# HAHHHD/mllp

Hardware: AMD Instinct MI355X
Metric: LP instances/sec (fwd+bwd) on Netlib batch; achieved HBM GB/s on CSR SpMM (higher is better)
Workload: dtype f32; 1 GPU; netlib_full: BASELINE.json configs[2], 97 instances / 1,074,147 nnz per global batch, one block-diagonal batch per GPU, one Adam step per global batch: fwd + BCE + bwd + gradient all-reduce + Adam, fp32; global_batch=97, instances_rank0=97, nnz_rank0=1074147, hip_graph=False, parallelism=dp1

## Files before the change

### mllp_amd/csrc/fused_kernels.hip

```cpp
#include <algorithm>
#include <vector>

#include "device_utils.h"
#include "host_graph.h"
#include "internal.h"
#include "node_bodies.h"

namespace mllp {

typedef float f32x4m __attribute__((ext_vector_type(4)));

#ifdef MLLP_TIMING_BUILD
static int g_fused_abl = [] {
    const char* e = getenv("MLLP_FUSED_ABL");
    return e ? atoi(e) : 0;
}();
#define FUSED_ABL(bit) ((J.abl & (bit)) != 0)
__device__ unsigned long long g_fused_stamps[8192 * 8];
__device__ unsigned long long g_fused_stamps1[8192 * 8];
#define FUSED_STAMP(k)                                                                      \
    {                                                                                       \
        __builtin_amdgcn_sched_barrier(0);                                                  \
        const unsigned long long now_ = __builtin_amdgcn_s_memtime();                       \
        __builtin_amdgcn_sched_barrier(0);                                                  \
// ... 1399 lines not shown
        }
    }
    const float x = J.x_dst[rowc];
    const float Zn = J.Z[rowc];
    const float4 ax = reinterpret_cast<const float4*>(J.aux)[rowc];
    {
        float* rt = tiles + 64 * G1S + lane * R1S;
        rt[0] = writer ? x : 0.0f;
        rt[1] = writer ? Zn : 0.0f;
        rt[2] = writer ? 1.0f : 0.0f;
        rt[3] = writer ? ax.w : 0.0f;
        rt[4] = writer ? ax.x : 0.0f;
    }
    const float Dn = gv * Zn + gb * ax.w + ge * ax.x;
    const float cc = gb - Dn;
    const float qp = fmaf(W.pq, x, W.pq0), t = fmaf(W.pt, x, W.pt0);
    float ds = 0.0f, dt = 0.0f, dq = 0.0f;
    const int n_mine = slot_count(r);
    FUSED_STAMP(1)
    for (int k0 = 0; __any(k0 < n_mine); k0 += 8) {
        Ent8 N;
        const bool more = __any(k0 + 8 < n_mine);
        if (more) ent8_load(J.s, r, k0 + 8, N);
#define MLLP_BWD1_SLOT(K, E_)                                                              \
    {                                                                                      \
        const float l_ = fmaf(qp, E_.y, E_.x * t);                                         \
        const float al_ = (K) < n_mine ? exp_acc(l_ - ax.y) * ax.z : 0.0f;                 \
        const float dl_ = al_ * fmaf(gv, E_.y, fmaf(E_.x, ge, cc));                        \
        ds += dl_;                                                                         \
        dt = fmaf(dl_, E_.x, dt);                                                          \
        dq = fmaf(dl_, E_.y, dq);                                                          \
    }
        MLLP_BWD1_SLOT(k0, E.e0)
        MLLP_BWD1_SLOT(k0 + 1, E.e1)
        MLLP_BWD1_SLOT(k0 + 2, E.e2)
        MLLP_BWD1_SLOT(k0 + 3, E.e3)
        if (__any(k0 + 4 < n_mine)) {
            MLLP_BWD1_SLOT(k0 + 4, E.e4)
            MLLP_BWD1_SLOT(k0 + 5, E.e5)
            MLLP_BWD1_SLOT(k0 + 6, E.e6)
            MLLP_BWD1_SLOT(k0 + 7, E.e7)
        }
#undef MLLP_BWD1_SLOT
        if (more) E = N;
    }
    FUSED_STAMP(2)
    if (r.mode >= 1) {
        ds = shared_sum1(ds, r.mode); dt = shared_sum1(dt, r.mode); dq = shared_sum1(dq, r.mode);
    }
    if (r.mode == 3) {
        const int wave = threadIdx.x >> 6;
        if (lane == 0) *reinterpret_cast<float4*>(merge_lds + wave * 4) = make_float4(ds, dt, dq, 0.0f);
        __syncthreads();
        float a = 0.0f, b = 0.0f, c = 0.0f;
        for (int w = 0; w < FW; ++w) {
            const float4 v = lds4(merge_lds + w * 4);
            a += v.x; b += v.y; c += v.z;
        }
        ds = a; dt = b; dq = c;
        __syncthreads();
        if (threadIdx.x >= 64) return;
    }
    if (writer) {
        accS[0] = fmaf(dq, x, accS[0]);
        accS[1] += dq;
        accS[2] = fmaf(ds, x, accS[2]);
        accS[3] = fmaf(dt, x, accS[3]);
        accS[4] += ds;
        accS[5] += dt;
    }
    FUSED_STAMP(3)
    const int kq = lane >> 4, rr = lane & 15;
    const float* gt = tiles + kq * G1S + rr;
    const float* rt = tiles + 64 * G1S + kq * R1S + rr;
#pragma unroll
    for (int s = 0; s < 16; ++s) {
        const float a = gt[4 * s * G1S];
        const float b = rr < 5 ? rt[4 * s * R1S] : 0.0f;
        accT = __builtin_amdgcn_mfma_f32_16x16x4f32(a, b, accT, 0, 0, 0);
    }
    FUSED_STAMP(4)
}

__global__ __launch_bounds__(FT) void fused_bwd1_kernel(BwdLaunch1 A) {
    __shared__ BwdW1 Ws_[MAXJOBS];
    __shared__ float merge_lds[FW * 4];
    __shared__ float tiles_[FW * TILE1];
    const int tid = threadIdx.x, lane = tid & 63, wave = tid >> 6;
    for (int j = 0; j < A.n_jobs; ++j) {
        const BwdJob1& J = A.job[j];
        BwdW1& W = Ws_[j];
        if (tid < 16) { W.wv[tid] = J.p.Wv[tid]; W.bv[tid] = J.p.bv[tid]; W.we[tid] = J.p.we[tid]; }
        if (tid == 0) { W.pq = J.D[OFF_PQ]; W.pq0 = J.D[OFF_PQ0]; W.pt = J.D[OFF_PT]; W.pt0 = J.D[OFF_PT0]; }
    }
    __syncthreads();
    float* tiles = tiles_ + wave * TILE1;
    const BlockPart B = block_part();
#ifdef MLLP_TIMING_BUILD
    unsigned long long stamp_sum[8] = {0, 0, 0, 0, 0, 0, 0, 0};
    unsigned long long stamp_last = __builtin_amdgcn_s_memtime();
    const unsigned long long stamp_begin = stamp_last;
#define STAMP_ARGS1 , stamp_sum, stamp_last
#else
#define STAMP_ARGS1
#endif
    for (int j = 0; j < A.n_jobs; ++j) {
        const BwdJob1& J = A.job[j];
        const PartTiers P = J.s.part[B.px];
        f32x4m accT = splat4(0.0f);
        float accS[6] = {0.0f, 0.0f, 0.0f, 0.0f, 0.0f, 0.0f};
        for (int k = B.bi; k < P.n_block; k += B.gp)
            bwd1_row(J, Ws_[j], block_slot<1>(J.s, P.row0 + k, tid), lane, merge_lds, tiles, accT, accS STAMP_ARGS1);
        WaveList wl = wave_list(J.s, B.px, B.gw);
        for (int c0 = 0; c0 < wl.L; c0 += 64) {
            wave_list_chunk(wl, c0, lane);
            int it = wave_list_get(wl, 0);
            SlotReq q = item_request<1>(J.s, P, max(it, 0), lane);
            for (int k = 0; it >= 0; ++k) {
                const int itn = wave_list_get(wl, k + 1);
                const RowSlot r = slot_make(q);
                q = item_request<1>(J.s, P, max(itn, 0), lane);
                bwd1_row(J, Ws_[j], r, lane, merge_lds, tiles, accT, accS STAMP_ARGS1);
#ifdef MLLP_TIMING_BUILD
                stamp_sum[7] += 1;
#endif
                it = itn;
            }
        }
        __syncthreads();
        float* red = tiles_;
#pragma unroll
        for (int q = 0; q < 4; ++q) red[wave * 262 + ((lane >> 4) * 4 + q) * 16 + (lane & 15)] = accT[q];
#pragma unroll
        for (int i = 0; i < 6; ++i) {
            const float v = wave_sum(accS[i]);
            if (lane == 0) red[wave * 262 + 256 + i] = v;
        }
        __syncthreads();
        float* dst = J.stats + (size_t)blockIdx.x * STAT_FLOATS;
        for (int i = tid; i < STAT_FLOATS; i += FT) dst[i] = 0.0f;
        __syncthreads();
        if (tid < 262) {
            float v = 0.0f;
            for (int w = 0; w < FW; ++w) v += red[w * 262 + tid];
            const int o = tid >> 4, n = tid & 15;
            if (tid >= 256) {
                const int i = tid - 256;
                const int slot = i == 0 ? 768 : i == 1 ? 1024 : i == 2 ? 1280 : i == 3 ? 1280 + 16 : i == 4 ? 1536 : 1536 + 16;
                dst[slot] = v;
            } else if (n == 0) dst[o * 16] = v;
            else if (n == 1) dst[256 + o * 16] = v;
            else if (n < 5) dst[512 + o * 16 + (n - 2)] = v;
        }
        __syncthreads();
#ifdef MLLP_TIMING_BUILD
        stamp_last = __builtin_amdgcn_s_memtime();
#endif
    }
#ifdef MLLP_TIMING_BUILD
    if (lane == 0) {
        stamp_sum[6] = __builtin_amdgcn_s_memtime() - stamp_begin;
        unsigned long long* d = g_fused_stamps1 + (size_t)(blockIdx.x * FW + wave) * 8;
        for (int k = 0; k < 8; ++k) d[k] = stamp_sum[k];
    }
#endif
#undef STAMP_ARGS1
}

__global__ __launch_bounds__(RT) void fused_head_bwd_kernel(int n, const float* __restrict__ h3, const float* __restrict__ fcw,
                                                            const float* __restrict__ dlogits, const int* __restrict__ perm,
                                                            float* __restrict__ dh3, float* __restrict__ head_part) {
    __shared__ float head_lds[(RT / 64) * 18];
    const int tid = threadIdx.x, lane = tid & 63, part = lane & 3;
    HeadAcc ha;
    ha.w = f4zero(); ha.b = 0.0f; ha.l = 0.0f;
    const float4 fw = ld4(fcw + 4 * part);
    for (int row = blockIdx.x * (RT / 4) + (tid >> 2); row < n; row += gridDim.x * (RT / 4)) {
        const float dz = dlogits[perm[row]];
        const float4 hv = ld4(h3 + (size_t)row * 16 + 4 * part);
        *reinterpret_cast<float4*>(dh3 + (size_t)row * 16 + 4 * part) = f4scale(fw, dz);
        fma4(dz, hv, ha.w);
        if (part == 0) ha.b += dz;
    }
    head_partials_store<RT / 64>(ha, head_lds, head_part, tid);
}

struct ReduceArgs {
    const float* stats[MODEL_CONVS];
    float* out[MODEL_CONVS];
    int nblk;
    const float* head_part;
    float* head_out;
    float* loss_out;
};

__device__ __forceinline__ void fused_reduce_body(const ReduceArgs& A, int n_conv) {
    __shared__ float sh[32][32];
    const int tid = threadIdx.x;
    if ((int)blockIdx.x == n_conv * STAT_TILES) {
        if (!A.head_part) return;
        const int col = tid & 31, slice = tid >> 5;
        float v = 0.0f;
        if (col < 18)
            for (int b = slice; b < A.nblk; b += 32) v += A.head_part[(size_t)b * 18 + col];
        sh[slice][col] = v;
        __syncthreads();
        if (tid < 18) {
            float t = 0.0f;
            for (int q = 0; q < 32; ++q) t += sh[q][tid];
            if (tid < 17) A.head_out[tid] = t;
            else if (A.loss_out) A.loss_out[0] = t;
        }
        return;
    }
    float* sh4 = &sh[0][0];
    const int col = tid & 255, slice = tid >> 8;
    const int c = blockIdx.x / STAT_TILES, tile = blockIdx.x % STAT_TILES;
    const float* src = A.stats[c] + tile * 256 + col;
    float v = 0.0f;
    int b = slice;
    for (; b + 124 < A.nblk; b += 128) {
        float t[32];
#pragma unroll
        for (int q = 0; q < 32; ++q) t[q] = src[(size_t)(b + 4 * q) * STAT_FLOATS];
#pragma unroll
        for (int q = 0; q < 32; ++q) v += t[q];
    }
    for (; b + 28 < A.nblk; b += 32) {
        float t[8];
#pragma unroll
        for (int q = 0; q < 8; ++q) t[q] = src[(size_t)(b + 4 * q) * STAT_FLOATS];
#pragma unroll
        for (int q = 0; q < 8; ++q) v += t[q];
    }
    for (; b < A.nblk; b += 4) v += src[(size_t)b * STAT_FLOATS];
    sh4[slice * 256 + col] = v;
    __syncthreads();
    if (tid < 256) A.out[c][tile * 256 + tid] = (sh4[tid] + sh4[256 + tid]) + (sh4[512 + tid] + sh4[768 + tid]);
}
__global__ __launch_bounds__(RT) void fused_reduce_kernel(ReduceArgs A, int n_conv) { fused_reduce_body(A, n_conv); }

struct TailArgs {
    ReduceArgs R;
    ConvParams p[MODEL_CONVS];
    int cin[MODEL_CONVS];
    float* grads[MODEL_CONVS];
    float* zero;
    int n_zero;
    float* params; const float* grads_all; float* m; float* v; float* state;
    float eps;
    int n_params;
    float* D[MODEL_CONVS];
    unsigned long long* sync;
    unsigned* err;
};
__device__ __forceinline__ bool tail_barrier(unsigned long long* cnt, unsigned long long target, unsigned* err_host) {
    __shared__ int ok_s;
    unsigned long long* err_dev = cnt + 2;
    __syncthreads();
    if (threadIdx.x == 0) {
        __threadfence();
        __hip_atomic_fetch_add(cnt, 1ull, __ATOMIC_RELEASE, __HIP_MEMORY_SCOPE_AGENT);
        int spins = 0;
        while (__hip_atomic_load(cnt, __ATOMIC_ACQUIRE, __HIP_MEMORY_SCOPE_AGENT) < target && ++spins < (1 << 22))
            __builtin_amdgcn_s_sleep(8);
        if (spins >= (1 << 22)) {
            __hip_atomic_store(err_dev, 1ull, __ATOMIC_RELAXED, __HIP_MEMORY_SCOPE_AGENT);
            __hip_atomic_store(err_host, 1u, __ATOMIC_RELAXED, __HIP_MEMORY_SCOPE_SYSTEM);
        }
        __threadfence();
        ok_s = __hip_atomic_load(err_dev, __ATOMIC_RELAXED, __HIP_MEMORY_SCOPE_AGENT) == 0ull;
    }
    __syncthreads();
    return ok_s != 0;
}
__global__ __launch_bounds__(RT) void fused_tail_kernel(TailArgs A, int n_conv) {
    const unsigned long long G = gridDim.x, epoch = A.sync[1];
    const int b = blockIdx.x;
    const float step = A.state[0] + 1.0f, lr = A.state[1], b1 = A.state[2], b2 = A.state[3];
    fused_reduce_body(A.R, n_conv);
    if (!tail_barrier(A.sync, (epoch + 1) * G, A.err)) return;
    if (b < n_conv) {
        finalize_conv_body(A.cin[b], A.p[b], A.R.out[b], 1, A.grads[b]);
        __syncthreads();
        const int off = (int)(A.grads[b] - A.grads_all), n = 4 * FEAT * A.cin[b] + 5 * FEAT;
        adam_slice(A.params + off, A.grads_all + off, A.m + off, A.v + off, step, lr, b1, b2, A.eps, 1.0f, n);
        __syncthreads();
        if (threadIdx.x < BLOCK) param_prep_body(A.p[b], A.cin[b], A.D[b]);
    } else if (b == n_conv) {
        for (int k = threadIdx.x; k < A.n_zero; k += RT) A.zero[k] = 0.0f;
        const int off = (int)(A.R.head_out - A.grads_all);
        adam_slice(A.params + off, A.grads_all + off, A.m + off, A.v + off, step, lr, b1, b2, A.eps, 1.0f, A.n_params - off);
        if (threadIdx.x == 0) {
            A.state[0] = step;
            A.sync[1] = epoch + 1;
        }
    }
}

__global__ __launch_bounds__(256) void fused_fill_kernel(int n_dst, const int* __restrict__ perm, const int* __restrict__ ptr,
                                                         const int* __restrict__ idx, const float* __restrict__ val,
                                                         const int* __restrict__ inv_src, const int* __restrict__ sptr,
                                                         int2* __restrict__ sent) {
    const int k = blockIdx.x * 4 + (threadIdx.x >> 6), lane = threadIdx.x & 63;
    if (k >= n_dst) return;
    const int r = perm[k], beg = ptr[r], deg = ptr[r + 1] - beg, o = sptr[k];
    for (int e = lane; e < deg; e += 64) sent[o + e] = make_int2(inv_src[idx[beg + e]], __float_as_int(val[beg + e]));
}
__global__ void fused_permute_kernel(int n, const int* __restrict__ perm, const float* __restrict__ src, float* __restrict__ dst) {
    for (int i = blockIdx.x * blockDim.x + threadIdx.x; i < n; i += gridDim.x * blockDim.x) dst[i] = src[perm[i]];
}
__global__ void fused_pregather_kernel(int64_t nnz, const int2* __restrict__ sent, const float* __restrict__ xs,
                                       float2* __restrict__ sax) {
    for (int64_t e = blockIdx.x * (int64_t)blockDim.x + threadIdx.x; e < nnz; e += (int64_t)gridDim.x * blockDim.x) {
        const int2 v = sent[e];
        sax[e] = make_float2(__int_as_float(v.y), xs[v.x]);
    }
}

#ifdef MLLP_TIMING_BUILD
extern "C" int mllp_timing_read_stamps(unsigned long long* host, int n) {
    return hipMemcpyFromSymbol(host, HIP_SYMBOL(g_fused_stamps), (size_t)n * sizeof(unsigned long long)) == hipSuccess ? 0 : -1;
}
extern "C" int mllp_timing_read_stamps1(unsigned long long* host, int n) {
    return hipMemcpyFromSymbol(host, HIP_SYMBOL(g_fused_stamps1), (size_t)n * sizeof(unsigned long long)) == hipSuccess ? 0 : -1;
}
#endif

template <class T>
static int dev_alloc(mllp_graph* g, size_t count, T** out, const T* host = nullptr, size_t room = 1) {
    void* p = nullptr;
    MLLP_HIP_TRY(hipMalloc(&p, std::max<size_t>(count, room) * sizeof(T)));
    if (count < room) MLLP_HIP_TRY(hipMemset(p, 0, room * sizeof(T)));
    g->allocs.push_back(p);
    if (host && count) MLLP_HIP_TRY(hipMemcpy(p, host, count * sizeof(T), hipMemcpyHostToDevice));
    *out = static_cast<T*>(p);
    return MLLP_OK;
}

static void set_tiers(FusedTiersDev& d, const FusedTiers& t) {
    d.n_block = t.n_block; d.n_wave = t.n_wave; d.n_group = t.n_group; d.n_base = t.n_base;
}

int fused_refill_values(mllp_graph* g, hipStream_t s) {
    int rc;
    if (g->M > 0) {
        hipLaunchKernelGGL(fused_fill_kernel, dim3((unsigned)((g->M + 3) / 4)), dim3(256), 0, s, (int)g->M, g->perm_c, g->A.ptr,
                           g->A.idx, g->A.val, g->inv_v, g->FA.sptr, reinterpret_cast<int2*>(g->FA.sent));
        if ((rc = check_launch("fused_fill A"))) return rc;
    }
    if (g->N > 0) {
        hipLaunchKernelGGL(fused_fill_kernel, dim3((unsigned)((g->N + 3) / 4)), dim3(256), 0, s, (int)g->N, g->perm_v, g->At.ptr,
                           g->At.idx, g->At.val, g->inv_c, g->FAt.sptr, reinterpret_cast<int2*>(g->FAt.sent));
        if ((rc = check_launch("fused_fill At"))) return rc;
    }
    return MLLP_OK;
}

int fused_graph_build(mllp_graph* g, const int* h_csr_ptr, const int* h_csc_ptr) {
    if (g->fused_built) return MLLP_OK;
    if ((int64_t)g->h_csr_ptr.size() != g->M + 1 && !h_csr_ptr) return fail(MLLP_EINVAL, "fused path: no host row pointers");
    HostFusedOrient hc, hv;
    {
#ifdef MLLP_SCALAR_PARTITION
        const std::vector<int> part = host_partition_instances(host_instance_cost(h_csr_ptr, g->h_inst_ptr_m),
                                                               host_instance_cost(h_csc_ptr, g->h_inst_ptr_n), FUSED_PARTS);
#else
        const std::vector<int> part = host_partition_instances_v(host_instance_loads(h_csr_ptr, g->h_inst_ptr_m),
                                                                 host_instance_loads(h_csc_ptr, g->h_inst_ptr_n), FUSED_PARTS);
#endif
        host_build_fused_orient(h_csr_ptr, (int)g->M, g->h_inst_ptr_m, part, &hc);
        host_build_fused_orient(h_csc_ptr, (int)g->N, g->h_inst_ptr_n, part, &hv);
    }
    int rc;
    if ((rc = dev_alloc(g, (size_t)g->M, &g->perm_c, hc.perm.data()))) return rc;
    if ((rc = dev_alloc(g, (size_t)g->N, &g->perm_v, hv.perm.data()))) return rc;
    if ((rc = dev_alloc(g, (size_t)g->M, &g->inv_c, hc.inv.data()))) return rc;
    if ((rc = dev_alloc(g, (size_t)g->N, &g->inv_v, hv.inv.data()))) return rc;
    FusedOrient& A = g->FA;
    FusedOrient& At = g->FAt;
    A.n_dst = (int)g->M; A.n_src = (int)g->N; A.nnz = (int)g->nnz;
    At.n_dst = (int)g->N; At.n_src = (int)g->M; At.nnz = (int)g->nnz;
    for (int q = 0; q < NP; ++q) {
        set_tiers(A.t16[q], hc.t16[q]); set_tiers(A.t1[q], hc.t1[q]);
        set_tiers(At.t16[q], hv.t16[q]); set_tiers(At.t1[q], hv.t1[q]);
    }
    for (int q = 0; q <= NP; ++q) { A.row0[q] = hc.row0[q]; At.row0[q] = hv.row0[q]; }
    {
        const int gp = fused_grid(g) / NP;
        const HostFusedOrient* ho[2] = {&hc, &hv};
        FusedOrient* dv[2] = {&A, &At};
        for (int k = 0; k < 2; ++k) {
            HostWaveLists l16, l16x2, l1;
            host_build_wave_lists(*ho[k], false, gp * FW, FW, 4, &l16);
            host_build_wave_lists(*ho[k], false, 2 * gp * FW, FW, 2, &l16x2);
            host_build_wave_lists(*ho[k], true, gp * FW, FW, 8, &l1);
            FusedOrient& d = *dv[k];
            d.L16 = l16.L; d.nw16 = l16.waves_per_part;
            d.L16x2 = l16x2.L; d.nw16x2 = l16x2.waves_per_part;
            d.L1 = l1.L; d.nw1 = l1.waves_per_part;
            if ((rc = dev_alloc(g, l16.order.size(), &d.lst16, l16.order.data()))) return rc;
            if ((rc = dev_alloc(g, l16x2.order.size(), &d.lst16x2, l16x2.order.data()))) return rc;
            if ((rc = dev_alloc(g, l1.order.size(), &d.lst1, l1.order.data()))) return rc;
        }
    }
    if ((rc = dev_alloc(g, (size_t)g->M + 1, &A.sptr, hc.sptr.data(), 2))) return rc;
    if ((rc = dev_alloc(g, (size_t)g->N + 1, &At.sptr, hv.sptr.data(), 2))) return rc;
    if ((rc = dev_alloc(g, (size_t)g->nnz * 2, &A.sent, (const int*)nullptr, 2))) return rc;
    if ((rc = dev_alloc(g, (size_t)g->nnz * 2, &At.sent, (const int*)nullptr, 2))) return rc;
    if ((rc = dev_alloc(g, (size_t)g->nnz * 2, &A.sax, (const float*)nullptr, 2))) return rc;
    if ((rc = dev_alloc(g, (size_t)g->nnz * 2, &At.sax, (const float*)nullptr, 2))) return rc;
    if ((rc = dev_alloc(g, (size_t)g->N, &g->inv_n_p))) return rc;
    if ((rc = dev_alloc(g, (size_t)g->N, &g->x1_p))) return rc;
    if ((rc = dev_alloc(g, (size_t)g->M, &g->x2_p))) return rc;
    if ((rc = dev_alloc(g, (size_t)g->N, &g->labels_p))) return rc;
    if (!g->tail_sync) {
        if ((rc = dev_alloc(g, (size_t)4, &g->tail_sync))) return rc;
        MLLP_HIP_TRY(hipMemset(g->tail_sync, 0, 32));
        MLLP_HIP_TRY(hipHostMalloc((void**)&g->tail_err_host, 64, hipHostMallocMapped));
        *g->tail_err_host = 0u;
        MLLP_HIP_TRY(hipHostGetDevicePointer((void**)&g->tail_err_dev, g->tail_err_host, 0));
    }
    if ((rc = fused_refill_values(g, 0))) return rc;
    if (g->N > 0) {
        hipLaunchKernelGGL(fused_permute_kernel, dim3(256), dim3(256), 0, 0, (int)g->N, g->perm_v, g->inv_n, g->inv_n_p);
        if ((rc = check_launch("fused_permute inv_n"))) return rc;
    }
    MLLP_HIP_TRY(hipDeviceSynchronize());
    g->fused_built = true;
    return MLLP_OK;
}

int fused_bind(mllp_graph* g, const float* x1, const float* x2, const float* labels, hipStream_t s) {
    int rc;
    hipStreamCaptureStatus cap = hipStreamCaptureStatusNone;
    (void)hipStreamIsCapturing(s, &cap);
    const bool capturing = cap != hipStreamCaptureStatusNone;
    if (capturing) g->bind_captured = true;
    if (g->bind_captured) g->bound_x1 = g->bound_x2 = g->bound_labels = nullptr;
    if (x1 != g->bound_x1 || x2 != g->bound_x2) {
        if (g->N > 0) hipLaunchKernelGGL(fused_permute_kernel, dim3(256), dim3(256), 0, s, (int)g->N, g->perm_v, x1, g->x1_p);
        if (g->M > 0) hipLaunchKernelGGL(fused_permute_kernel, dim3(256), dim3(256), 0, s, (int)g->M, g->perm_c, x2, g->x2_p);
        if (g->nnz > 0) {
            hipLaunchKernelGGL(fused_pregather_kernel, dim3(1024), dim3(256), 0, s, g->nnz,
                               reinterpret_cast<const int2*>(g->FA.sent), g->x1_p, reinterpret_cast<float2*>(g->FA.sax));
            hipLaunchKernelGGL(fused_pregather_kernel, dim3(1024), dim3(256), 0, s, g->nnz,
                               reinterpret_cast<const int2*>(g->FAt.sent), g->x2_p, reinterpret_cast<float2*>(g->FAt.sax));
        }
        if ((rc = check_launch("fused_bind inputs"))) return rc;
        if (!capturing) { g->bound_x1 = x1; g->bound_x2 = x2; }
    }
    if (labels && labels != g->bound_labels) {
        if (g->N > 0) hipLaunchKernelGGL(fused_permute_kernel, dim3(256), dim3(256), 0, s, (int)g->N, g->perm_v, labels, g->labels_p);
        if ((rc = check_launch("fused_bind labels"))) return rc;
        if (!capturing) g->bound_labels = labels;
    }
    return MLLP_OK;
}

int fused_grid(const mllp_graph* g) { return std::max(std::min(g->n_cu, STAT_BLOCKS_MAX) / NP, 1) * NP; }

static FwdJob16 fwd_job16(const FusedOrient& o, const FusedModel& m, int c, const float* x_src, const float* x_dst, float* h) {
    const ConvWs& w = m.w.c[c];
    FwdJob16 J = {};
    J.s = items_dev(o, 0);
    J.x_src = x_src; J.x_dst = x_dst; J.D = w.derived; J.p = conv_params_at(conv_at(m.P, c), MODEL_CONV[c].cin);
    J.h = h; J.Z = w.Z; J.aux = w.aux;
    J.head = 0;
#ifdef MLLP_TIMING_BUILD
    J.abl = g_fused_abl;
#endif
    return J;
}
static FwdJob1 fwd_job1(const FusedOrient& o, const FusedModel& m, int c, const float* x_dst, float* h) {
    const ConvWs& w = m.w.c[c];
    FwdJob1 J = {};
    J.s = items_dev(o, 1);
    J.x_dst = x_dst; J.D = w.derived; J.p = conv_params_at(conv_at(m.P, c), MODEL_CONV[c].cin);
    J.h = h; J.Z = w.Z; J.aux = w.aux;
    return J;
}

static FwdJob16 l3_fwd_job(const mllp_graph* g, const FusedModel& m, int head_mode) {
    const ModelWs& w = m.w;
    FwdJob16 J = fwd_job16(g->FAt, m, CONV_3V, w.h2c, w.h2v, w.h3v);
    J.head = head_mode;
    J.fcw = m.P + OFF_FC; J.fcb = m.P + OFF_FC + FEAT; J.inv_n = g->inv_n_p; J.labels = g->labels_p; J.perm = g->perm_v;
    J.inv_batch = m.inv_batch;
    J.logits = m.logits; J.head_part = w.head_partials;
    return J;
}

int fused_forward(mllp_graph* g, const FusedModel& m, int head_mode, hipStream_t s, bool skip_prep) {
    const int G = fused_grid(g);
    const ModelWs& w = m.w;
    int rc;
    if ((rc = fused_bind(g, m.x1, m.x2, head_mode == 2 ? m.labels : nullptr, s))) return rc;
    if (!skip_prep && (rc = model_param_prep(m.P, w, s))) return rc;
    {
        FwdLaunch1 L = {};
        L.n_jobs = 2;
        L.job[0] = fwd_job1(g->FAt, m, CONV_1V, g->x1_p, w.h1v);
        L.job[1] = fwd_job1(g->FA, m, CONV_1C, g->x2_p, w.h1c);
        hipLaunchKernelGGL(fused_fwd1_kernel, dim3(G), dim3(FT), 0, s, L);
// ... 45 lines not shown
static SrcJob16 src_job16(const FusedOrient& o_src_major, const ConvWs& w, const float* x_rows, float* dx, const float* add) {
    SrcJob16 J = {};
    J.s = items_dev(o_src_major, 2);
    J.x = x_rows; J.rec = w.rec; J.dx = dx;
    J.addp = add ? add : x_rows; J.addw = add ? 1.0f : 0.0f; J.mask = 1;
    return J;
}
static BwdJob1 bwd_job1(const FusedOrient& o, const FusedModel& m, int c, const float* x_dst, const float* g_masked) {
    const ConvWs& w = m.w.c[c];
    BwdJob1 J = {};
    J.s = items_dev(o, 1);
    J.x_dst = x_dst; J.D = w.derived; J.p = conv_params_at(conv_at(m.P, c), MODEL_CONV[c].cin);
    J.g = g_masked; J.Z = w.Z; J.aux = w.aux; J.stats = w.stats;
    return J;
}

int fused_backward(const mllp_graph* g, const FusedModel& m, bool premasked, float* grads, float* loss, hipStream_t s,
                   const FusedAdam* adam) {
    const int G = fused_grid(g);
    const ModelWs& w = m.w;
    int rc;
    const FusedOrient& A = g->FA;
    const FusedOrient& At = g->FAt;
    if (premasked) {
        L3Job L = {};
        L.f = l3_fwd_job(g, m, 2);
        L.rec = w.c[CONV_3V].rec; L.dx_dst = w.d2v; L.stats = w.c[CONV_3V].stats;
        hipLaunchKernelGGL(fused_l3_kernel, dim3(G), dim3(FT), 0, s, L);
        if ((rc = check_launch("fused_l3"))) return rc;
    } else {
        BwdLaunch16 L = {};
        L.n_jobs = 1;
        L.job[0] = bwd_job16(At, m, CONV_3V, w.h2c, w.h2v, w.h3v, w.d3v, nullptr, w.d2v, true, true);
        hipLaunchKernelGGL(fused_bwd16_kernel, dim3(G), dim3(FT), 0, s, L);
        if ((rc = check_launch("fused_bwd16 C3"))) return rc;
    }
    {
        SrcLaunch16 S = {};
        S.n_jobs = 1;
        S.job[0] = src_job16(A, w.c[CONV_3V], w.h2c, w.d2c, nullptr);
        hipLaunchKernelGGL(fused_src16_kernel, dim3(2 * G), dim3(FT), 0, s, S);
        if ((rc = check_launch("fused_src16 C3"))) return rc;
        BwdLaunch16 L = {};
        L.n_jobs = 1;
        L.job[0] = bwd_job16(At, m, CONV_2V, w.h1c, w.h1v, nullptr, w.d2v, nullptr, w.d1v, true, true);
        hipLaunchKernelGGL(fused_bwd16_kernel, dim3(G), dim3(FT), 0, s, L);
        if ((rc = check_launch("fused_bwd16 C2V"))) return rc;
    }
    {
        BwdLaunch16 L = {};
        L.n_jobs = 1;
        L.job[0] = bwd_job16(A, m, CONV_2C, w.h1v, w.h1c, nullptr, w.d2c, nullptr, w.d1c, true, true);
        hipLaunchKernelGGL(fused_bwd16_kernel, dim3(G), dim3(FT), 0, s, L);
        if ((rc = check_launch("fused_bwd16 C2C"))) return rc;
        SrcLaunch16 S = {};
        S.n_jobs = 2;
        S.job[0] = src_job16(A, w.c[CONV_2V], w.h1c, w.d1c_b, w.d1c);
        S.job[1] = src_job16(At, w.c[CONV_2C], w.h1v, w.d1v_b, w.d1v);
        hipLaunchKernelGGL(fused_src16_kernel, dim3(2 * G), dim3(FT), 0, s, S);
        if ((rc = check_launch("fused_src16 C2V + C2C"))) return rc;
    }
    {
        BwdLaunch1 L = {};
        L.n_jobs = 2;
        L.job[0] = bwd_job1(A, m, CONV_1C, g->x2_p, w.d1c_b);
        L.job[1] = bwd_job1(At, m, CONV_1V, g->x1_p, w.d1v_b);
        hipLaunchKernelGGL(fused_bwd1_kernel, dim3(G), dim3(FT), 0, s, L);
        if ((rc = check_launch("fused_bwd1"))) return rc;
    }
    ReduceArgs R = {};
    for (int c = 0; c < MODEL_CONVS; ++c) { R.stats[c] = w.c[c].stats; R.out[c] = w.c[c].red; }
    R.nblk = G;
    R.head_part = w.head_partials;
    R.head_out = grads + OFF_FC;
    R.loss_out = loss;
    if (adam) {
        TailArgs T = {};
        T.R = R;
        for (int c = 0; c < MODEL_CONVS; ++c) {
            T.p[c] = conv_params_at(conv_at(m.P, c), MODEL_CONV[c].cin);
            T.cin[c] = MODEL_CONV[c].cin;
            T.grads[c] = conv_at(grads, c);
            T.D[c] = w.c[c].derived;
        }
        T.zero = grads + OFF_UNUSED;
        T.n_zero = LEN_UNUSED;
        T.params = adam->params; T.grads_all = grads; T.m = adam->m; T.v = adam->v; T.state = adam->state;
        T.eps = adam->eps;
        T.n_params = adam->n;
        T.sync = g->tail_sync;
        T.err = g->tail_err_dev;
        if (g->tail_err_host && *(volatile unsigned*)g->tail_err_host != 0u)
            return fail(MLLP_EHIP, "the grid barrier of fused_tail_kernel timed out in an earlier step (the device was shared with "
                                   "other work): parameters and optimizer state since then are invalid; recreate the graph");
        hipLaunchKernelGGL(fused_tail_kernel, dim3(MODEL_CONVS * STAT_TILES + 1), dim3(RT), 0, s, T, MODEL_CONVS);
        return check_launch("fused_tail");
    }
    {
        hipLaunchKernelGGL(fused_reduce_kernel, dim3(MODEL_CONVS * STAT_TILES + 1), dim3(RT), 0, s, R, MODEL_CONVS);
        if ((rc = check_launch("fused_reduce"))) return rc;
    }
    return model_finalize(g, m.P, w, true, grads, s);
}

}
```

### mllp_amd/csrc/graph.cpp

```cpp
#include <algorithm>
#include <atomic>
#include <cmath>
#include <cstring>

#include "host_graph.h"
#include "internal.h"

namespace mllp {

static thread_local std::string g_err;
void set_error(const std::string& msg) { g_err = msg; }
int fail(int code, const std::string& msg) {
    g_err = msg;
    return code;
}
int hip_fail(hipError_t e, const char* what) {
    g_err = std::string(what) + ": " + hipGetErrorString(e);
    return e == hipErrorOutOfMemory ? MLLP_ENOMEM : MLLP_EHIP;
}
const char* last_error_cstr() { return g_err.c_str(); }

static std::atomic<int64_t> g_fused_grid_limit{0};

template <class T>
// ... 118 lines not shown
    if (rc) {
        std::string keep = mllp_last_error();
        mllp_graph_destroy(g);
        set_error(keep);
        return rc;
    }
    *out = g;
    return MLLP_OK;
}

extern "C" int mllp_graph_create_device(int64_t n_inst, const int64_t* inst_ptr_m, const int64_t* inst_ptr_n,
                                        int64_t nnz, const int32_t* d_csr_ptr, const int32_t* d_csr_idx,
                                        const float* d_csr_val, const int32_t* d_csc_ptr, const int32_t* d_csc_idx,
                                        const float* d_csc_val, int32_t tier_wave, int32_t tier_block, void* stream,
                                        mllp_graph_t** out) {
    if (!out) return fail(MLLP_EINVAL, "mllp_graph_create_device: out is null");
    *out = nullptr;
    if (n_inst <= 0 || !inst_ptr_m || !inst_ptr_n || !d_csr_ptr || !d_csc_ptr || nnz < 0)
        return fail(MLLP_EINVAL, "mllp_graph_create_device: bad arguments");
    if (nnz > 0 && (!d_csr_idx || !d_csr_val || !d_csc_idx || !d_csc_val))
        return fail(MLLP_EINVAL, "mllp_graph_create_device: null index/value arrays");
    int64_t M = inst_ptr_m[n_inst], N = inst_ptr_n[n_inst];
    if (nnz >= INT32_MAX - 1 || M >= INT32_MAX - 1 || N >= INT32_MAX - 1)
        return fail(MLLP_ERANGE, "batch exceeds int32 indexing");
    hipStream_t s = (hipStream_t)stream;
    mllp_graph* g = new mllp_graph();
    g->M = M; g->N = N; g->nnz = nnz; g->n_inst = n_inst;
    g->h_inst_ptr_m.assign(inst_ptr_m, inst_ptr_m + n_inst + 1);
    g->h_inst_ptr_n.assign(inst_ptr_n, inst_ptr_n + n_inst + 1);
    g->tier_wave = tier_wave;
    g->tier_block = tier_block;
    choose_tiers(g);
    g->A.n_dst = (int)M; g->A.n_src = (int)N;
    g->At.n_dst = (int)N; g->At.n_src = (int)M;
    auto dcopy = [&](const void* src, size_t bytes, void** dst) -> int {
        void* p = nullptr;
        MLLP_HIP_TRY(hipMalloc(&p, std::max<size_t>(bytes, 4)));
        g->allocs.push_back(p);
        if (bytes) MLLP_HIP_TRY(hipMemcpyAsync(p, src, bytes, hipMemcpyDeviceToDevice, s));
        *dst = p;
        return MLLP_OK;
    };
    int rc = MLLP_OK;
    std::vector<int> h_rp(M + 1), h_cp(N + 1);
    do {
        if ((rc = dcopy(d_csr_ptr, (M + 1) * 4, (void**)&g->A.ptr))) break;
        if ((rc = dcopy(d_csr_idx, nnz * 4, (void**)&g->A.idx))) break;
        if ((rc = dcopy(d_csr_val, nnz * 4, (void**)&g->A.val))) break;
        if ((rc = dcopy(d_csc_ptr, (N + 1) * 4, (void**)&g->At.ptr))) break;
        if ((rc = dcopy(d_csc_idx, nnz * 4, (void**)&g->At.idx))) break;
        if ((rc = dcopy(d_csc_val, nnz * 4, (void**)&g->At.val))) break;
        hipError_t e = hipMemcpyAsync(h_rp.data(), d_csr_ptr, (M + 1) * 4, hipMemcpyDeviceToHost, s);
        if (e == hipSuccess) e = hipMemcpyAsync(h_cp.data(), d_csc_ptr, (N + 1) * 4, hipMemcpyDeviceToHost, s);
        if (e == hipSuccess) e = hipStreamSynchronize(s);
        if (e != hipSuccess) { rc = hip_fail(e, "copy row pointers to host"); break; }
        if (h_rp[0] != 0 || h_cp[0] != 0 || h_rp[M] != nnz || h_cp[N] != nnz) {
            rc = fail(MLLP_EINVAL, "row pointers inconsistent with nnz");
            break;
        }
        if ((rc = build_tiers(g, g->A, h_rp.data()))) break;
        if ((rc = build_tiers(g, g->At, h_cp.data()))) break;
        if ((rc = finish_common(g))) break;
        g->h_csr_ptr = h_rp; g->h_csc_ptr = h_cp;
        if (g->nnz < ((int64_t)32 << 20) && (rc = fused_graph_build(g, h_rp.data(), h_cp.data()))) break;
    } while (0);
    if (rc) {
        std::string keep = mllp_last_error();
        mllp_graph_destroy(g);
        set_error(keep);
        return rc;
    }
    *out = g;
    return MLLP_OK;
}

extern "C" int mllp_graph_destroy(mllp_graph_t* g) {
    if (!g) return MLLP_OK;
    for (mllp::Orient* o : {&g->A, &g->At}) {
        for (mllp::StreamCopy& sc : o->stream) mllp::stream_copy_free(sc);
        mllp::lane_copy_free(o->lane1);
        for (mllp::Tiled& tl : o->tiled) mllp::tiled_free(tl);
    }
    for (void* p : g->allocs) (void)hipFree(p);
    if (g->tail_err_host) (void)hipHostFree(g->tail_err_host);
    for (auto& e : g->ev)
        if (e) (void)hipEventDestroy(e);
    if (g->aux) (void)hipStreamDestroy(g->aux);
    delete g;
    return MLLP_OK;
}

extern "C" int mllp_graph_dims(const mllp_graph_t* g, int64_t dims[12]) {
    if (!g || !dims) return fail(MLLP_EINVAL, "mllp_graph_dims: null argument");
    dims[0] = g->M; dims[1] = g->N; dims[2] = g->nnz; dims[3] = g->n_inst;
    dims[4] = g->A.n_group; dims[5] = g->A.n_wave; dims[6] = g->A.n_chunk;
    dims[7] = g->At.n_group; dims[8] = g->At.n_wave; dims[9] = g->At.n_chunk;
    dims[10] = g->A.n_split; dims[11] = g->At.n_split;
    return MLLP_OK;
}

extern "C" int mllp_set_fused_grid_limit(int64_t workgroups, int64_t* previous) {
    if (workgroups < 0) return fail(MLLP_EINVAL, "mllp_set_fused_grid_limit: the limit must be 0 (none) or a positive number of workgroups");
    const int64_t old = g_fused_grid_limit.exchange(workgroups, std::memory_order_relaxed);
    if (previous) *previous = old;
    return MLLP_OK;
}

extern "C" int mllp_graph_fused_grid(const mllp_graph_t* g, int64_t info[4]) {
    if (!g || !info) return fail(MLLP_EINVAL, "mllp_graph_fused_grid: null argument");
    info[0] = fused_grid(g); info[1] = FUSED_PARTS; info[2] = g->n_cu_dev; info[3] = g->grid_limit;
    return MLLP_OK;
}

extern "C" int mllp_graph_export(const mllp_graph_t* g, int which, void* host_dst, int64_t capacity_bytes) {
    if (!g || !host_dst) return fail(MLLP_EINVAL, "mllp_graph_export: null argument");
    const void* src = nullptr;
    int64_t bytes = 0;
    switch (which) {
        case 0: src = g->A.ptr; bytes = (g->M + 1) * 4; break;
        case 1: src = g->A.idx; bytes = g->nnz * 4; break;
        case 2: src = g->A.val; bytes = g->nnz * 4; break;
        case 3: src = g->At.ptr; bytes = (g->N + 1) * 4; break;
        case 4: src = g->At.idx; bytes = g->nnz * 4; break;
        case 5: src = g->At.val; bytes = g->nnz * 4; break;
        case 6: src = g->inv_n; bytes = g->N * 4; break;
        default: return fail(MLLP_EINVAL, "mllp_graph_export: unknown array id");
    }
    if (capacity_bytes < bytes) return fail(MLLP_EINVAL, "mllp_graph_export: destination too small");
    MLLP_HIP_TRY(hipDeviceSynchronize());
    if (bytes) MLLP_HIP_TRY(hipMemcpy(host_dst, src, bytes, hipMemcpyDeviceToHost));
    return MLLP_OK;
}
```

### mllp_amd/csrc/internal.h

```cpp
#pragma once
#include <hip/hip_runtime.h>
#include <stdint.h>

#include <algorithm>
#include <string>
#include <vector>

#include "../../include/mllp_hip.h"

namespace mllp {

constexpr int FEAT = 16;
constexpr int BLOCK = 256;
constexpr int REC_W = 40;
constexpr int STAT_TILES = 7;
constexpr int STAT_FLOATS = STAT_TILES * 256;
constexpr int STAT_BLOCKS_MAX = 256;

void set_error(const std::string& msg);
int fail(int code, const std::string& msg);
int hip_fail(hipError_t e, const char* what);

#define MLLP_HIP_TRY(expr)                                              \
    do {                                                                \
// ... 55 lines not shown
    int64_t nnz = 0;
    int* tile_row = nullptr;
    int* tile_blk = nullptr;
    int* tile_col = nullptr;
    int* rows = nullptr;
    int* whdr = nullptr;
    unsigned* offs = nullptr;
    float* vals = nullptr;
    int* vmap = nullptr;
    double build_seconds = 0.0;
};

struct CopyArray {
    void** p;
    int64_t bytes;
};
enum { SC_TILE_BLK, SC_BLK_ID, SC_ROWS, SC_ENT, SC_TILE_ROW, SC_HDR };
enum { LC_TILE_BLK, LC_TILE_COL, LC_ROWS, LC_OFFS, LC_TILE_ROW, LC_WHDR, LC_VALS };
enum { TL_TILE_BLK, TL_BLK_ID, TL_PTR2, TL_PERM, TL_ENT };
std::vector<CopyArray> stream_copy_arrays(StreamCopy& sc, int geom);
std::vector<CopyArray> lane_copy_arrays(LaneCopy& lc);
std::vector<CopyArray> tiled_arrays(Tiled& tl, int variant, int64_t nnz);
int copy_alloc(const CopyArray& a);
void copy_free(const std::vector<CopyArray>& arrays);

struct Orient {
    LaneCopy lane1;
    StreamCopy stream[4];
    Tiled tiled[TILED_VARIANTS];
    int n_dst = 0, n_src = 0;
    int* ptr = nullptr;
    int* idx = nullptr;
    float* val = nullptr;
    int* rows_group = nullptr;
    int* rows_wave = nullptr;
    int* chunks = nullptr;
    int* split = nullptr;
    int n_group = 0, n_wave = 0, n_chunk = 0, n_split = 0, n_slots = 0;
    float* scratch = nullptr;
    int tier_wave = 0;
    bool short_rows = false;
};
struct FusedTiersDev {
    int n_block = 0, n_wave = 0, n_group = 0, n_base = 0;
};
constexpr int FUSED_NP = 8;
struct FusedOrient {
    int n_dst = 0, n_src = 0, nnz = 0;
    int* sptr = nullptr;
    int* sent = nullptr;
    float* sax = nullptr;
    int row0[FUSED_NP + 1] = {};
    FusedTiersDev t16[FUSED_NP], t1[FUSED_NP];
    int* lst16 = nullptr; int* lst16x2 = nullptr; int* lst1 = nullptr;
    int L16 = 0, L16x2 = 0, L1 = 0, nw16 = 0, nw16x2 = 0, nw1 = 0;
};
constexpr int SCRATCH_NS = 20;

}

struct mllp_graph {
    int64_t M = 0, N = 0, nnz = 0, n_inst = 0;
    mllp::Orient A;
    mllp::Orient At;
    float* inv_n = nullptr;
    int* inst_ptr_n = nullptr;
    int* inst_ptr_m = nullptr;
    std::vector<int64_t> h_inst_ptr_n, h_inst_ptr_m;
    std::vector<int> h_csr_ptr, h_csc_ptr;
    int tier_wave = 0, tier_block = 0, chunk_nnz = 0;
    int max_inst_n = 0;
    int n_cu = 256;
    int n_cu_dev = 256;
    int64_t grid_limit = 0;
    int path = 0;
    bool fused_built = false;
    mllp::FusedOrient FA, FAt;
    int* perm_v = nullptr;
    int* perm_c = nullptr;
    int* inv_v = nullptr;
    int* inv_c = nullptr;
    float* inv_n_p = nullptr;
    unsigned long long* tail_sync = nullptr;
    unsigned* tail_err_host = nullptr;
    unsigned* tail_err_dev = nullptr;
    float* x1_p = nullptr;
    float* x2_p = nullptr;
    float* labels_p = nullptr;
    const void* bound_x1 = nullptr;
    const void* bound_x2 = nullptr;
    const void* bound_labels = nullptr;
    bool bind_captured = false;
    int ws_path = -1;
    const void* ws_ptr = nullptr;
    const void* ws_params = nullptr;
    const void* folded_ws = nullptr;
    const void* folded_params = nullptr;
    int* at_pos = nullptr;
    float* scale_buf = nullptr;
    float* norm_scale = nullptr;
    int* plant_ws = nullptr;
    hipStream_t aux = nullptr;
    hipEvent_t ev[16] = {};
    std::vector<void*> allocs;
};

namespace mllp {

inline void forget_forward(mllp_graph* g) {
    g->ws_ptr = g->ws_params = nullptr;
    g->ws_path = -1;
}

template <class T>
inline int graph_alloc_once(mllp_graph* g, T*& slot, size_t bytes) {
    if (slot) return MLLP_OK;
    void* p = nullptr;
    MLLP_HIP_TRY(hipMalloc(&p, bytes));
    g->allocs.push_back(p);
    slot = static_cast<T*>(p);
    return MLLP_OK;
}

struct ConvParams {
    const float *Wk, *bk, *Wq, *bq, *Wv, *bv, *we, *Ws, *bs;
};
constexpr int conv_param_count(int cin) { return 4 * FEAT * cin + 5 * FEAT; }

enum { CONV_1V, CONV_1C, CONV_2V, CONV_2C, CONV_3V };
constexpr int MODEL_CONVS = CONV_3V + 1;
struct ConvSpec {
    bool dst_is_var;
    int cin;
};
constexpr ConvSpec MODEL_CONV[MODEL_CONVS] = {{true, 1}, {false, 1}, {true, 16}, {false, 16}, {true, 16}};
struct ConvOffsets {
    int at[MODEL_CONVS + 1];
};
constexpr ConvOffsets conv_offsets() {
    ConvOffsets o = {};
    for (int c = 0; c < MODEL_CONVS; ++c) o.at[c + 1] = o.at[c] + conv_param_count(MODEL_CONV[c].cin);
    return o;
}
constexpr ConvOffsets CONV_OFF = conv_offsets();
constexpr int OFF_UNUSED = CONV_OFF.at[MODEL_CONVS], LEN_UNUSED = conv_param_count(FEAT);
constexpr int OFF_FC = OFF_UNUSED + LEN_UNUSED;
constexpr int NUM_PARAMS = OFF_FC + FEAT + 1;
static_assert(CONV_OFF.at[CONV_1V] == 0 && CONV_OFF.at[CONV_1C] == 144 && CONV_OFF.at[CONV_2V] == 288 &&
                  CONV_OFF.at[CONV_2C] == 1392 && CONV_OFF.at[CONV_3V] == 2496,
              "conv offsets differ from GNNModel.state_dict()");
static_assert(OFF_UNUSED == 3600 && LEN_UNUSED == 1104 && OFF_FC == 4704, "gconv3_s2w / fc offsets differ from state_dict()");
static_assert(NUM_PARAMS == MLLP_NUM_PARAMS, "the layout's total differs from MLLP_NUM_PARAMS");
template <class T>
inline T* conv_at(T* base, int c) { return base + CONV_OFF.at[c]; }

inline ConvParams conv_params_at(const float* base, int cin) {
    ConvParams p;
    const float* q = base;
    p.Wk = q; q += FEAT * cin;
    p.bk = q; q += FEAT;
    p.Wq = q; q += FEAT * cin;
    p.bq = q; q += FEAT;
    p.Wv = q; q += FEAT * cin;
    p.bv = q; q += FEAT;
    p.we = q; q += FEAT;
    p.Ws = q; q += FEAT * cin;
    p.bs = q;
    return p;
// ... 165 lines not shown
```

Before: 312,700 instances/s.

## Replace tail grid barrier with per-conv last-block tickets and split reductions

```diff
diff --git a/mllp_amd/csrc/fused_kernels.hip b/mllp_amd/csrc/fused_kernels.hip
--- a/mllp_amd/csrc/fused_kernels.hip
+++ b/mllp_amd/csrc/fused_kernels.hip
@@ -1505,6 +1505,39 @@
     FUSED_STAMP(4)
 }
 
+__host__ __device__ constexpr int bwd1_stat_slot(int tid) {
+    const int o = tid >> 4, n = tid & 15;
+    if (tid >= 256) {
+        const int i = tid - 256;
+        return i == 0 ? 768 : i == 1 ? 1024 : i == 2 ? 1280 : i == 3 ? 1280 + 16 : i == 4 ? 1536 : i == 5 ? 1536 + 16 : -1;
+    }
+    if (n == 0) return o * 16;
+    if (n == 1) return 256 + o * 16;
+    if (n < 5) return 512 + o * 16 + (n - 2);
+    return -1;
+}
+constexpr int L1_STAT_N = 86;
+__host__ __device__ constexpr int l1_stat_tid(int k) {
+    return k < 16 ? 16 * k : k < 32 ? 16 * (k - 16) + 1 : k < 80 ? 16 * ((k - 32) / 3) + 2 + (k - 32) % 3 : 256 + (k - 80);
+}
+constexpr int L1_STAT_COLS[L1_STAT_N] = {
+    0, 16, 32, 48, 64, 80, 96, 112, 128, 144, 160, 176, 192, 208, 224, 240,
+    256, 272, 288, 304, 320, 336, 352, 368, 384, 400, 416, 432, 448, 464, 480, 496,
+    512, 513, 514, 528, 529, 530, 544, 545, 546, 560, 561, 562, 576, 577, 578, 592, 593, 594, 608, 609, 610, 624, 625, 626,
+    640, 641, 642, 656, 657, 658, 672, 673, 674, 688, 689, 690, 704, 705, 706, 720, 721, 722, 736, 737, 738, 752, 753, 754,
+    768, 1024, 1280, 1296, 1536, 1552};
+constexpr bool l1_stat_cols_match() {
+    int n = 0;
+    for (int t = 0; t < 262; ++t) n += bwd1_stat_slot(t) >= 0;
+    if (n != L1_STAT_N) return false;
+    for (int k = 0; k < L1_STAT_N; ++k)
+        if (L1_STAT_COLS[k] != bwd1_stat_slot(l1_stat_tid(k))) return false;
+    for (int k = 1; k < L1_STAT_N; ++k)
+        if (L1_STAT_COLS[k] <= L1_STAT_COLS[k - 1]) return false;
+    return true;
+}
+static_assert(l1_stat_cols_match(), "L1_STAT_COLS must list the slots that fused_bwd1_kernel stores");
+
 __global__ __launch_bounds__(FT) void fused_bwd1_kernel(BwdLaunch1 A) {
     __shared__ BwdW1 Ws_[MAXJOBS];
     __shared__ float merge_lds[FW * 4];
@@ -1566,14 +1599,8 @@
         if (tid < 262) {
             float v = 0.0f;
             for (int w = 0; w < FW; ++w) v += red[w * 262 + tid];
-            const int o = tid >> 4, n = tid & 15;
-            if (tid >= 256) {
-                const int i = tid - 256;
-                const int slot = i == 0 ? 768 : i == 1 ? 1024 : i == 2 ? 1280 : i == 3 ? 1280 + 16 : i == 4 ? 1536 : 1536 + 16;
-                dst[slot] = v;
-            } else if (n == 0) dst[o * 16] = v;
-            else if (n == 1) dst[256 + o * 16] = v;
-            else if (n < 5) dst[512 + o * 16 + (n - 2)] = v;
+            const int slot = bwd1_stat_slot(tid);
+            if (slot >= 0) dst[slot] = v;
         }
         __syncthreads();
 #ifdef MLLP_TIMING_BUILD
@@ -1663,6 +1690,20 @@
 }
 __global__ __launch_bounds__(RT) void fused_reduce_kernel(ReduceArgs A, int n_conv) { fused_reduce_body(A, n_conv); }
 
+constexpr int TAIL_QUARTERS = 4;
+constexpr int TAIL_UNITS16 = STAT_TILES * TAIL_QUARTERS;
+constexpr int TAIL_FINISH = MODEL_CONVS;
+constexpr int TAIL_SYNC_WORDS = 8;
+static_assert(TAIL_FINISH < TAIL_SYNC_WORDS, "one counter per conv and the finish counter");
+constexpr int TAIL_STAGE = conv_param_count(FEAT);
+constexpr int TAIL_STAGE_PER_THREAD = (TAIL_STAGE + RT - 1) / RT;
+__device__ __forceinline__ ConvParams tail_rebase(const ConvParams& p, const float* from, const float* to) {
+    ConvParams q;
+    q.Wk = to + (p.Wk - from); q.bk = to + (p.bk - from); q.Wq = to + (p.Wq - from); q.bq = to + (p.bq - from);
+    q.Wv = to + (p.Wv - from); q.bv = to + (p.bv - from); q.we = to + (p.we - from); q.Ws = to + (p.Ws - from);
+    q.bs = to + (p.bs - from);
+    return q;
+}
 struct TailArgs {
     ReduceArgs R;
     ConvParams p[MODEL_CONVS];
@@ -1674,51 +1715,130 @@
     float eps;
     int n_params;
     float* D[MODEL_CONVS];
+    int n16, conv16[MODEL_CONVS];
+    int n1, conv1[MODEL_CONVS];
     unsigned long long* sync;
-    unsigned* err;
-};
-__device__ __forceinline__ bool tail_barrier(unsigned long long* cnt, unsigned long long target, unsigned* err_host) {
-    __shared__ int ok_s;
-    unsigned long long* err_dev = cnt + 2;
+};
+template <int N>
+__device__ __forceinline__ void tail_slice_batch(const float* __restrict__ src, int& b, int nblk, float& v) {
+    for (; b + 4 * (N - 1) < nblk; b += 4 * N) {
+        float t[N];
+#pragma unroll
+        for (int q = 0; q < N; ++q) t[q] = src[(size_t)(b + 4 * q) * STAT_FLOATS];
+#pragma unroll
+        for (int q = 0; q < N; ++q) v += t[q];
+    }
+}
+__device__ __forceinline__ float tail_slice_sum(const float* __restrict__ src, int slice, int nblk) {
+    float v = 0.0f;
+    int b = slice;
+    tail_slice_batch<64>(src, b, nblk, v);
+    tail_slice_batch<16>(src, b, nblk, v);
+    tail_slice_batch<4>(src, b, nblk, v);
+    tail_slice_batch<1>(src, b, nblk, v);
+    return v;
+}
+__device__ __forceinline__ void tail_unit16(const float* __restrict__ stats, float* __restrict__ out, int nblk, int col0,
+                                            float* sh) {
+    const int tid = threadIdx.x;
+    if (tid < 4 * 64) sh[tid] = tail_slice_sum(stats + col0 + (tid & 63), tid >> 6, nblk);
+    __syncthreads();
+    if (tid < 64) out[col0 + tid] = (sh[tid] + sh[64 + tid]) + (sh[128 + tid] + sh[192 + tid]);
+}
+__device__ __forceinline__ void tail_unit1(const float* __restrict__ stats, float* __restrict__ out, int nblk, float* sh) {
+    const int tid = threadIdx.x, k = tid & 127, slice = tid >> 7;
+    const int slot = bwd1_stat_slot(l1_stat_tid(k < L1_STAT_N ? k : 0));
+    if (tid < 4 * 128 && k < L1_STAT_N) sh[slice * 128 + k] = tail_slice_sum(stats + slot, slice, nblk);
+    __syncthreads();
+    if (tid < L1_STAT_N) out[slot] = (sh[tid] + sh[128 + tid]) + (sh[256 + tid] + sh[384 + tid]);
+}
+__device__ __forceinline__ void tail_unit_fc(const ReduceArgs& A, float* sh) {
+    const int tid = threadIdx.x, col = tid & 31, slice = tid >> 5;
+    float v = 0.0f;
+    if (col < 18)
+        for (int b = slice; b < A.nblk; b += 32) v += A.head_part[(size_t)b * 18 + col];
+    sh[slice * 32 + col] = v;
+    __syncthreads();
+    if (tid < 18) {
+        float t = 0.0f;
+        for (int q = 0; q < 32; ++q) t += sh[q * 32 + tid];
+        if (tid < 17) A.head_out[tid] = t;
+        else if (A.loss_out) A.loss_out[0] = t;
+    }
+}
+__device__ __forceinline__ bool tail_ticket(unsigned long long* cnt, unsigned units, int* last_s) {
+    asm volatile("s_waitcnt vmcnt(0)" ::: "memory");
     __syncthreads();
     if (threadIdx.x == 0) {
-        __threadfence();
-        __hip_atomic_fetch_add(cnt, 1ull, __ATOMIC_RELEASE, __HIP_MEMORY_SCOPE_AGENT);
-        int spins = 0;
-        while (__hip_atomic_load(cnt, __ATOMIC_ACQUIRE, __HIP_MEMORY_SCOPE_AGENT) < target && ++spins < (1 << 22))
-            __builtin_amdgcn_s_sleep(8);
-        if (spins >= (1 << 22)) {
-            __hip_atomic_store(err_dev, 1ull, __ATOMIC_RELAXED, __HIP_MEMORY_SCOPE_AGENT);
-            __hip_atomic_store(err_host, 1u, __ATOMIC_RELAXED, __HIP_MEMORY_SCOPE_SYSTEM);
-        }
-        __threadfence();
-        ok_s = __hip_atomic_load(err_dev, __ATOMIC_RELAXED, __HIP_MEMORY_SCOPE_AGENT) == 0ull;
+        __builtin_amdgcn_fence(__ATOMIC_RELEASE, "agent");
+        asm volatile("s_waitcnt vmcnt(0)" ::: "memory");
+        const unsigned long long old = __hip_atomic_fetch_add(cnt, 1ull, __ATOMIC_RELAXED, __HIP_MEMORY_SCOPE_AGENT);
+        const int last = (old + 1ull) % units == 0ull;
+        if (last) {
+            __builtin_amdgcn_fence(__ATOMIC_ACQUIRE, "agent");
+            asm volatile("s_waitcnt vmcnt(0)" ::: "memory");
+        }
+        *last_s = last;
     }
     __syncthreads();
-    return ok_s != 0;
+    return *last_s != 0;
+}
+__device__ __forceinline__ void tail_finish(unsigned long long* cnt, unsigned finishers, float* state, float step) {
+    __syncthreads();
+    if (threadIdx.x == 0) {
+        const unsigned long long old = __hip_atomic_fetch_add(cnt, 1ull, __ATOMIC_RELAXED, __HIP_MEMORY_SCOPE_AGENT);
+        if ((old + 1ull) % finishers == 0ull) state[0] = step;
+    }
 }
 __global__ __launch_bounds__(RT) void fused_tail_kernel(TailArgs A, int n_conv) {
-    const unsigned long long G = gridDim.x, epoch = A.sync[1];
-    const int b = blockIdx.x;
-    const float step = A.state[0] + 1.0f, lr = A.state[1], b1 = A.state[2], b2 = A.state[3];
-    fused_reduce_body(A.R, n_conv);
-    if (!tail_barrier(A.sync, (epoch + 1) * G, A.err)) return;
-    if (b < n_conv) {
-        finalize_conv_body(A.cin[b], A.p[b], A.R.out[b], 1, A.grads[b]);
+    __shared__ float sh[32 * 32];
+    __shared__ int last_s;
+    const int b = blockIdx.x, n_units16 = A.n16 * TAIL_UNITS16;
+    int c;
+    if (b < n_units16) {
+        c = A.conv16[b / TAIL_UNITS16];
+        const int u = b % TAIL_UNITS16;
+        tail_unit16(A.R.stats[c], A.R.out[c], A.R.nblk, (u / TAIL_QUARTERS) * 256 + (u % TAIL_QUARTERS) * 64, sh);
+        if (!tail_ticket(A.sync + c, TAIL_UNITS16, &last_s)) return;
+    } else if (b < n_units16 + A.n1) {
+        c = A.conv1[b - n_units16];
+        tail_unit1(A.R.stats[c], A.R.out[c], A.R.nblk, sh);
         __syncthreads();
-        const int off = (int)(A.grads[b] - A.grads_all), n = 4 * FEAT * A.cin[b] + 5 * FEAT;
-        adam_slice(A.params + off, A.grads_all + off, A.m + off, A.v + off, step, lr, b1, b2, A.eps, 1.0f, n);
+    } else {
+        const float step = A.state[0] + 1.0f, lr = A.state[1], b1 = A.state[2], b2 = A.state[3];
+        tail_unit_fc(A.R, sh);
+        for (int k = threadIdx.x; k < A.n_zero; k += RT) A.zero[k] = 0.0f;
         __syncthreads();
-        if (threadIdx.x < BLOCK) param_prep_body(A.p[b], A.cin[b], A.D[b]);
-    } else if (b == n_conv) {
-        for (int k = threadIdx.x; k < A.n_zero; k += RT) A.zero[k] = 0.0f;
         const int off = (int)(A.R.head_out - A.grads_all);
         adam_slice(A.params + off, A.grads_all + off, A.m + off, A.v + off, step, lr, b1, b2, A.eps, 1.0f, A.n_params - off);
-        if (threadIdx.x == 0) {
-            A.state[0] = step;
-            A.sync[1] = epoch + 1;
-        }
-    }
+        tail_finish(A.sync + TAIL_FINISH, (unsigned)n_conv + 1u, A.state, step);
+        return;
+    }
+    __shared__ float stage[4][TAIL_STAGE];
+    float *g_l = stage[0], *p_l = stage[1], *m_l = stage[2], *v_l = stage[3];
+    const float step = A.state[0] + 1.0f, lr = A.state[1], b1 = A.state[2], b2 = A.state[3];
+    const int tid = threadIdx.x, off = (int)(A.grads[c] - A.grads_all), n = 4 * FEAT * A.cin[c] + 5 * FEAT;
+    float pr[TAIL_STAGE_PER_THREAD], mr[TAIL_STAGE_PER_THREAD], vr[TAIL_STAGE_PER_THREAD];
+#pragma unroll
+    for (int q = 0; q < TAIL_STAGE_PER_THREAD; ++q) {
+        const int i = off + min(tid + q * RT, n - 1);
+        pr[q] = A.params[i]; mr[q] = A.m[i]; vr[q] = A.v[i];
+    }
+    finalize_conv_body(A.cin[c], A.p[c], A.R.out[c], 1, g_l);
+#pragma unroll
+    for (int q = 0; q < TAIL_STAGE_PER_THREAD; ++q) {
+        const int i = tid + q * RT;
+        if (i < n) { p_l[i] = pr[q]; m_l[i] = mr[q]; v_l[i] = vr[q]; }
+    }
+    __syncthreads();
+    for (int i = tid; i < n; i += RT) A.grads[c][i] = g_l[i];
+    adam_slice(p_l, g_l, m_l, v_l, step, lr, b1, b2, A.eps, 1.0f, n);
+    __syncthreads();
+    for (int i = tid; i < n; i += RT) {
+        A.params[off + i] = p_l[i]; A.m[off + i] = m_l[i]; A.v[off + i] = v_l[i];
+    }
+    if (tid < BLOCK) param_prep_body(tail_rebase(A.p[c], A.p[c].Wk, p_l), A.cin[c], A.D[c]);
+    tail_finish(A.sync + TAIL_FINISH, (unsigned)n_conv + 1u, A.state, step);
 }
 
 __global__ __launch_bounds__(256) void fused_fill_kernel(int n_dst, const int* __restrict__ perm, const int* __restrict__ ptr,
@@ -1838,11 +1958,8 @@
     if ((rc = dev_alloc(g, (size_t)g->M, &g->x2_p))) return rc;
     if ((rc = dev_alloc(g, (size_t)g->N, &g->labels_p))) return rc;
     if (!g->tail_sync) {
-        if ((rc = dev_alloc(g, (size_t)4, &g->tail_sync))) return rc;
-        MLLP_HIP_TRY(hipMemset(g->tail_sync, 0, 32));
-        MLLP_HIP_TRY(hipHostMalloc((void**)&g->tail_err_host, 64, hipHostMallocMapped));
-        *g->tail_err_host = 0u;
-        MLLP_HIP_TRY(hipHostGetDevicePointer((void**)&g->tail_err_dev, g->tail_err_host, 0));
+        if ((rc = dev_alloc(g, (size_t)TAIL_SYNC_WORDS, &g->tail_sync))) return rc;
+        MLLP_HIP_TRY(hipMemset(g->tail_sync, 0, TAIL_SYNC_WORDS * sizeof(unsigned long long)));
     }
     if ((rc = fused_refill_values(g, 0))) return rc;
     if (g->N > 0) {
@@ -2054,6 +2171,8 @@
             T.cin[c] = MODEL_CONV[c].cin;
             T.grads[c] = conv_at(grads, c);
             T.D[c] = w.c[c].derived;
+            if (MODEL_CONV[c].cin == FEAT) T.conv16[T.n16++] = c;
+            else T.conv1[T.n1++] = c;
         }
         T.zero = grads + OFF_UNUSED;
         T.n_zero = LEN_UNUSED;
@@ -2061,11 +2180,7 @@
         T.eps = adam->eps;
         T.n_params = adam->n;
         T.sync = g->tail_sync;
-        T.err = g->tail_err_dev;
-        if (g->tail_err_host && *(volatile unsigned*)g->tail_err_host != 0u)
-            return fail(MLLP_EHIP, "the grid barrier of fused_tail_kernel timed out in an earlier step (the device was shared with "
-                                   "other work): parameters and optimizer state since then are invalid; recreate the graph");
-        hipLaunchKernelGGL(fused_tail_kernel, dim3(MODEL_CONVS * STAT_TILES + 1), dim3(RT), 0, s, T, MODEL_CONVS);
+        hipLaunchKernelGGL(fused_tail_kernel, dim3(T.n16 * TAIL_UNITS16 + T.n1 + 1), dim3(RT), 0, s, T, MODEL_CONVS);
         return check_launch("fused_tail");
     }
     {
diff --git a/mllp_amd/csrc/graph.cpp b/mllp_amd/csrc/graph.cpp
--- a/mllp_amd/csrc/graph.cpp
+++ b/mllp_amd/csrc/graph.cpp
@@ -224,7 +224,6 @@
         for (mllp::Tiled& tl : o->tiled) mllp::tiled_free(tl);
     }
     for (void* p : g->allocs) (void)hipFree(p);
-    if (g->tail_err_host) (void)hipHostFree(g->tail_err_host);
     for (auto& e : g->ev)
         if (e) (void)hipEventDestroy(e);
     if (g->aux) (void)hipStreamDestroy(g->aux);
diff --git a/mllp_amd/csrc/internal.h b/mllp_amd/csrc/internal.h
--- a/mllp_amd/csrc/internal.h
+++ b/mllp_amd/csrc/internal.h
@@ -161,8 +161,6 @@
     int* inv_c = nullptr;
     float* inv_n_p = nullptr;
     unsigned long long* tail_sync = nullptr;
-    unsigned* tail_err_host = nullptr;
-    unsigned* tail_err_dev = nullptr;
     float* x1_p = nullptr;
     float* x2_p = nullptr;
     float* labels_p = nullptr;
```

After: 314,700 instances/s, median of 6. About the same (+0.7%).
